# Mikubill/sketch2img

Hardware: AMD Instinct MI355X
Metric: sketch-guided images/sec whole-node, SD1.5 512px 50-step DDIM (higher is better)
Workload: dtype fp16

## Files before the change

include/skg.h:

```cpp
#ifndef SKG_H_
#define SKG_H_

#include <stddef.h>
#include <stdint.h>

#ifdef __cplusplus
extern "C" {
#endif

#define SKG_OK 0
#define SKG_E_BADARG (-1)
#define SKG_E_UNSUPPORTED (-2)
#define SKG_E_LAUNCH (-3)

#define SKG_ABI_VERSION 6
int skg_abi_version(void);
const char* skg_last_error(void);

#define SKG_EPI_RELU 1u
#define SKG_EPI_OUT_F32 2u
#define SKG_EPI_GEGLU 4u
#define SKG_EPI_BIAS_ROWS 8u

int skg_gemm_f16(const void* A, int lda, const void* B, int ldb, void* C, void* C_lo, int ldc, int M, int N, int K,
// ... 90 lines not shown
                  float alpha, float beta, void* stream);
int skg_batch_copy_f16(const void* In, int ldi, int in_batch_rows, void* Out, int ldo, int out_batch_rows,
                       int batches, int rows_per_batch, int C, void* stream);
int skg_silu_f16(const void* X, int ldx, void* Y, int ldy, int M, int C, void* stream);
int skg_quick_gelu_f16(const void* X, int ldx, void* Y, int ldy, int M, int C, void* stream);
int skg_quick_gelu_bwd_f16(const void* F, int ldf, const void* dY, int lddy, void* out, int ldo, int M, int C, void* stream);
int skg_gelu_f16(const void* X, int ldx, void* Y, int ldy, int M, int C, void* stream);
int skg_sumpool2x2_f16(const void* X, int ldx, void* Y, int ldy, int rows, int H, int W, int C,
                       void* stream);
int skg_nchw_f32_to_nhwc_f16(const float* X, void* Y, int rows, int C, int HW, int Cpad, void* stream);
int skg_nhwc_f16_to_nchw_f32(const void* X, int ldx, float* Y, int rows, int C, int HW, void* stream);

typedef struct {
  const float* P;
  int s;
  int pad_;
} SkgLgpTap;
int skg_lgp_layer0_gather(const SkgLgpTap* taps, int ntaps, const void* Wextra, int ldw,
                          const void* bias0, const float* noise, float sigma, int samples,
                          void* Z, int rows, int h, int w, int H0, void* stream);
int skg_lgp_layer0_scatter(const void* dZ, int lddz, void* dP, int rows, int h, int w, int s, int H0,
                           void* stream);
size_t skg_bn_scratch_floats(int samples, int C);
int skg_bn_stats(const void* X, int ldx, int samples, int segs, int seg_rows, int C, float eps,
                 float* stats, float* scratch, float* running_mean, float* running_var,
                 void* stream);
int skg_bn_stats_from_running(const float* running_mean, const float* running_var, int samples,
                              int C, float eps, float* stats, void* stream);
int skg_bn_apply(const void* X, int ldx, void* Y, int ldy, int samples, int segs, int seg_rows,
                 int C, const float* stats, const void* gamma, const void* beta, void* stream);
int skg_bn_relu_bwd(const void* X, int ldx, const void* dY, int lddy, void* dX, int lddx,
                    int samples, int segs, int seg_rows, int C, const float* stats,
                    const void* gamma, int train_mode, float* scratch, void* stream);
int skg_lgp_mse_seed(const void* out, int ldo, const float* target, void* dOut, int ldd,
                     float* loss, int samples, int h, int w, float loss_scale, void* stream);

size_t skg_colsum_scratch_floats(int C);
int skg_colsum_f16(const void* X, int ldx, int M, int C, float scale, float* out, float* scratch, void* stream);
int skg_bn_param_grads(const void* X, int ldx, const void* dY, int lddy, int rows, int C, const float* stats,
                       float scale, float* dgamma, float* dbeta, float* scratch, void* stream);
int skg_lgp_extra_features(const float* noise, float sigma, int samples, int rows, int h, int w, void* E, int ld,
                           void* stream);
int skg_lgp_mse_train(const void* out, int ldo, const float* target, void* dOut, int ldd, float* loss_parts,
                      int samples, int h, float loss_scale, void* stream);
int skg_adamw_step(float* param, const float* grad, float* exp_avg, float* exp_avg_sq, void* param_f16, size_t n,
                   float lr, float beta1, float beta2, float eps, float weight_decay, int step, float inv_grad_scale,
                   void* stream);
int skg_nonfinite_flag(const float* x, size_t n, float* flag, int reset, void* stream);
int skg_adamw_step_guarded(float* param, const float* grad, float* exp_avg, float* exp_avg_sq, void* param_f16, size_t n,
                           float lr, float beta1, float beta2, float eps, float weight_decay, int step,
                           float inv_grad_scale, const float* skip_flag, void* stream);

int skg_cfg_ddim_step(const void* eps_u, const void* eps_c, int ld, int lo_off, const float* x, float* x_prev,
                      float* eps_out, int samples, int HW, float g, float c0, float c1, float c2,
                      float c3, int vpred, void* stream);
int skg_cfg_ddim_eta_step(const void* eps_u, const void* eps_c, int ld, int lo_off, const float* x, const float* z,
                          float* x_prev, float* eps_out, int samples, int HW, float g, float c0, float c1,
                          float c2, float c_dir, float sigma, int vpred, void* stream);
int skg_softmax_rows_f16(const void* x, int ldx, void* y, int ldy, int M, int N, void* stream);
int skg_image_postprocess(const void* x, int ld, float* out, size_t pixels, int C, float scale, float shift,
                          void* stream);

int skg_image_to_u8(const void* x, int ld, void* out, size_t pixels, int C, float scale, float shift, void* stream);

int skg_gaussian_sample(const void* moments, int ld, const float* noise, float* out, int samples, int L, int HW,
                        float scale, void* stream);
// ... 32 lines not shown
```

sketch2img_amd/_lib.py:

```python
from __future__ import annotations

import ctypes
import os

import torch

_HERE = os.path.dirname(os.path.abspath(__file__))
LIB_PATH = os.environ.get("SKG_LIB") or os.path.join(_HERE, "libskg.so")

ABI_VERSION = 6

SIGNATURES = {
    "skg_abi_version": ("i", ""),
    "skg_last_error": ("s", ""),
    "skg_gemm_f16": ("i", "pipippiiiipppifupiip"),
    "skg_conv3x3_up2_f16": ("i", "pipppiiiiiiipp"),
    "skg_conv3x3_sc_f16": ("i", "pipiipppiiiiiipupip"),
    "skg_conv4x4s2_f16": ("i", "pippiiiiiipp"),
    "skg_conv3x3_wino_v_bytes": ("z", "iiii"),
    "skg_conv3x3_wino_f16": ("i", "pippppiiiiiipppiup"),
    "skg_groupnorm_wino_fwd": ("i", "pipiiiiifppipp"),
    "skg_gemm_f16_rows": ("i", "pipipiiiipiip"),
    "skg_gemm_gn_fused": ("i", "iiiiiii"),
    "skg_gemm_f16_geglu_keep": ("i", "pipipipiiiipp"),
# ... 30 lines not shown
    "skg_bn_scratch_floats": ("z", "ii"),
    "skg_bn_stats": ("i", "piiiiifppppp"),
    "skg_bn_stats_from_running": ("i", "ppiifpp"),
    "skg_bn_apply": ("i", "pipiiiiipppp"),
    "skg_bn_relu_bwd": ("i", "pipipiiiiippipp"),
    "skg_colsum_scratch_floats": ("z", "i"),
    "skg_colsum_f16": ("i", "piiifppp"),
    "skg_bn_param_grads": ("i", "pipiiipfpppp"),
    "skg_lgp_extra_features": ("i", "pfiiiipip"),
    "skg_lgp_mse_train": ("i", "pippipiifp"),
    "skg_adamw_step": ("i", "pppppzfffffifp"),
    "skg_lgp_mse_seed": ("i", "pippipiiifp"),
    "skg_cfg_ddim_step": ("i", "ppiipppiifffffip"),
    "skg_cfg_ddim_eta_step": ("i", "ppiippppiiffffffip"),
    "skg_softmax_rows_f16": ("i", "pipiiip"),
    "skg_image_postprocess": ("i", "pipziffp"),
    "skg_image_to_u8": ("i", "pipziffp"),
    "skg_gaussian_sample": ("i", "pippiiifp"),
    "skg_cfg_dpmpp2m_step": ("i", "ppiippppiiffffffip"),
    "skg_guidance_update": ("i", "pipppiifp"),
    "skg_box_probe_mfma": ("i", "pip"),
    "skg_instnorm_scratch_floats": ("z", "iii"),
    "skg_instnorm_act_f16": ("i", "piiiifipifpifpp"),
    "skg_convt4x4s2_f16": ("i", "pippiiiiiipip"),
    "skg_a2s_patch_f16": ("i", "ppiiiip"),
    "skg_a2s_tail": ("i", "pippiiip"),
    "skg_wgrad_scratch_floats": ("z", "iii"),
    "skg_wgrad_f16": ("i", "pipiiiifipppp"),
    "skg_layernorm_param_scratch_floats": ("z", "i"),
    "skg_layernorm_param_grads": ("i", "pipiiipfipppp"),
    "skg_quick_gelu_bwd_f16": ("i", "pipipiiip"),
    "skg_nonfinite_flag": ("i", "pzpip"),
    "skg_adamw_step_guarded": ("i", "pppppzfffffifpp"),
}

_CT = {"p": ctypes.c_void_p, "i": ctypes.c_int, "f": ctypes.c_float, "u": ctypes.c_uint,
       "z": ctypes.c_size_t, "s": ctypes.c_char_p}


class SkgTap(ctypes.Structure):
    _fields_ = [("P", ctypes.c_void_p), ("s", ctypes.c_int), ("pad_", ctypes.c_int)]


class SkgError(RuntimeError):
    rc = 0


def _load():
    if not os.path.exists(LIB_PATH):
        raise ImportError(
            f"{LIB_PATH} not found: build it with `python -c 'import __graft_entry__ as g; g.build()'` "
            "or `make -C sketch2img_amd/csrc`.  sketch2img_amd has no fallback compute path.")
    lib = ctypes.CDLL(LIB_PATH)
    for name, (ret, args) in SIGNATURES.items():
        try:
            fn = getattr(lib, name)
        except AttributeError as e:
            raise ImportError(f"libskg.so does not export {name}") from e
        fn.restype = _CT[ret]
        fn.argtypes = [_CT[a] for a in args]
    if lib.skg_abi_version() != ABI_VERSION:
        raise ImportError(f"{LIB_PATH}: ABI version {lib.skg_abi_version()}, this package binds version {ABI_VERSION} "
                          "(include/skg.h SKG_ABI_VERSION) - rebuild with `make -C sketch2img_amd/csrc`")
    return lib


# ... 13 lines not shown
```

sketch2img_amd/csrc/lgp.hip:

```cpp
#include "common.h"

namespace {

constexpr int BN_CHUNKS = 64;
constexpr int MAX_TAPS = 12;
constexpr int NEXTRA = 40;

struct TapArgs {
  const float* P[MAX_TAPS];
  int s[MAX_TAPS];
  int n;
};

__device__ __forceinline__ void bil_coord(int d, int s, int h, int& i0, int& i1, float& w1) {
  const float scale = (float)s / (float)h;
  float src = ((float)d + 0.5f) * scale - 0.5f;
  if (src < 0.f) src = 0.f;
  i0 = (int)src;
  if (i0 > s - 1) i0 = s - 1;
  i1 = i0 + (i0 < s - 1 ? 1 : 0);
  w1 = src - (float)i0;
}

__global__ __launch_bounds__(256) void lgp_gather_kernel(const TapArgs taps, const half_t* __restrict__ Wx, int ldw,
// ... 548 lines not shown
    v[i] = vi;
    float w = p[i] * (1.f - lr * wd);
    w -= lr * (mi / bc1) / (sqrtf(vi / bc2) + eps);
    p[i] = w;
    if (p16) p16[i] = (half_t)w;
  }
}

__device__ __forceinline__ unsigned nonfinite_bits(unsigned u) { return (u & 0x7f800000u) == 0x7f800000u; }
__device__ __forceinline__ unsigned nonfinite_bits(const uint4& u) {
  return nonfinite_bits(u.x) | nonfinite_bits(u.y) | nonfinite_bits(u.z) | nonfinite_bits(u.w);
}

__global__ __launch_bounds__(256) void nonfinite_flag_kernel(const unsigned* __restrict__ x, size_t n, size_t head,
                                                             size_t nvec, float* __restrict__ flag) {
  const uint4* __restrict__ xv = reinterpret_cast<const uint4*>(x + head);
  const size_t stride = (size_t)gridDim.x * 256;
  size_t i = (size_t)blockIdx.x * 256 + threadIdx.x;
  unsigned bad = 0;
  for (; i + 3 * stride < nvec; i += 4 * stride) {
    const uint4 a = xv[i], b = xv[i + stride], c = xv[i + 2 * stride], d = xv[i + 3 * stride];
    bad |= nonfinite_bits(a) | nonfinite_bits(b) | nonfinite_bits(c) | nonfinite_bits(d);
  }
  for (; i < nvec; i += stride) bad |= nonfinite_bits(xv[i]);
  if (blockIdx.x == 0) {
    const size_t body_end = head + 4 * nvec;
    if (threadIdx.x < head) bad |= nonfinite_bits(x[threadIdx.x]);
    if (threadIdx.x >= 64 && body_end + (threadIdx.x - 64) < n) bad |= nonfinite_bits(x[body_end + (threadIdx.x - 64)]);
  }
  const unsigned long long hits = __ballot(bad != 0);
  if (hits != 0 && (threadIdx.x & 63) == 0) *flag = 1.0f;
}

inline int ew_grid(size_t total_items) {
  size_t b = (total_items + 255) / 256;
  if (b > 4096) b = 4096;
  if (b < 1) b = 1;
  return (int)b;
}

}

static inline bool tap_fits(int s, int h, int w) {
  return s > 0 && h % s == 0 && ((long long)s * w) % h == 0 && w % (int)((long long)s * w / h) == 0;
}

static inline bool grid_ok(int h, int w) { return h == w || (h % GT == 0 && w % GT == 0); }

extern "C" int skg_lgp_layer0_gather(const SkgLgpTap* taps, int ntaps, const void* Wextra, int ldw, const void* bias0,
                                     const float* noise, float sigma, int samples, void* Z, int rows, int h, int w, int H0,
                                     void* stream) {
  SKG_REQUIRE(grid_ok(h, w));
  SKG_REQUIRE(taps && ntaps > 0 && ntaps <= MAX_TAPS && bias0 && noise && Z && rows > 0 && h > 0 && w > 0);
  SKG_REQUIRE(H0 % 4 == 0 && skg_aligned(Z, 8) && samples > 0 && rows % samples == 0);
  SKG_REQUIRE(Wextra ? (ldw % 8 == 0 && skg_aligned(Wextra, 16)) : (h % GT == 0 && w % GT == 0 && H0 % GC == 0));
  TapArgs a{};
  a.n = ntaps;
  for (int i = 0; i < ntaps; ++i) {
    SKG_REQUIRE(taps[i].P && tap_fits(taps[i].s, h, w) && skg_aligned(taps[i].P, 16));
    a.P[i] = taps[i].P;
    a.s[i] = taps[i].s;
  }
  if (h % GT == 0 && w % GT == 0 && H0 % GC == 0) {
    hipLaunchKernelGGL(lgp_gather_tiled_kernel, dim3((h / GT) * (w / GT), rows, H0 / GC), dim3(256), 0,
                       (hipStream_t)stream, a, (const half_t*)Wextra, ldw, (const half_t*)bias0, noise, sigma, samples,
                       (half_t*)Z, rows, h, w, H0);
// ... 73 lines not shown
extern "C" int skg_bn_apply(const void* X, int ldx, void* Y, int ldy, int samples, int segs, int seg_rows, int C,
                            const float* stats, const void* gamma, const void* beta, void* stream) {
  SKG_REQUIRE(X && Y && stats && gamma && beta && samples > 0 && C % 8 == 0 && ldx % 8 == 0 && ldy % 8 == 0);
  SKG_REQUIRE(skg_aligned(X, 16) && skg_aligned(Y, 16) && skg_aligned(gamma, 16) && skg_aligned(beta, 16));
  SKG_REQUIRE(segs > 0 && seg_rows > 0);
  hipLaunchKernelGGL((bn_apply_kernel<0>), dim3(bn_apply_chunks(segs * seg_rows, C), samples), dim3(256), 0, (hipStream_t)stream,
                     (const half_t*)X, ldx, (const half_t*)nullptr, 0, (half_t*)Y, ldy, samples, segs, seg_rows, C,
                     stats, (const float*)nullptr, (const half_t*)gamma, (const half_t*)beta, 1);
  SKG_CHECK_LAUNCH("skg_bn_apply");
  return SKG_OK;
}

extern "C" int skg_bn_relu_bwd(const void* X, int ldx, const void* dY, int lddy, void* dX, int lddx, int samples,
                               int segs, int seg_rows, int C, const float* stats, const void* gamma,
                               int train_mode, float* scratch, void* stream) {
  SKG_REQUIRE(X && dY && dX && stats && gamma && scratch && samples > 0 && C % 8 == 0);
  SKG_REQUIRE(ldx % 8 == 0 && lddy % 8 == 0 && lddx % 8 == 0 && skg_aligned(X, 16) && skg_aligned(dY, 16) &&
              skg_aligned(dX, 16) && skg_aligned(gamma, 16));
  hipStream_t st = (hipStream_t)stream;
  float* sums = scratch + (size_t)samples * BN_CHUNKS * C * 2;
  if (train_mode) {
    hipLaunchKernelGGL((bn_partial_kernel<1>), dim3(BN_CHUNKS, samples), dim3(256), 0, st, (const half_t*)X, ldx,
                       (const half_t*)dY, lddy, samples, segs, seg_rows, C, stats, scratch);
    hipLaunchKernelGGL((bn_finalize_kernel<1>), dim3(skg_cdiv(C, 128), samples), dim3(128), 0, st, scratch, samples, C,
                       segs * seg_rows, 0.f, sums, (float*)nullptr);
  }
  hipLaunchKernelGGL((bn_apply_kernel<1>), dim3(bn_apply_chunks(segs * seg_rows, C), samples), dim3(256), 0, st, (const half_t*)X, ldx,
                     (const half_t*)dY, lddy, (half_t*)dX, lddx, samples, segs, seg_rows, C, stats, sums,
                     (const half_t*)gamma, (const half_t*)nullptr, train_mode);
  SKG_CHECK_LAUNCH("skg_bn_relu_bwd");
  return SKG_OK;
}

extern "C" size_t skg_colsum_scratch_floats(int C) { return (size_t)CS_CHUNKS * C; }

extern "C" int skg_colsum_f16(const void* X, int ldx, int M, int C, float scale, float* out, float* scratch,
                              void* stream) {
  SKG_REQUIRE(X && out && scratch && M > 0 && C > 0 && C % 8 == 0 && ldx % 8 == 0 && ldx >= C && skg_aligned(X, 16));
  hipStream_t st = (hipStream_t)stream;
  hipLaunchKernelGGL(colsum_partial_kernel, dim3(C / 8, CS_CHUNKS), dim3(256), 0, st, (const half_t*)X, ldx, M, C,
                     scratch);
  hipLaunchKernelGGL(colsum_final_kernel, dim3(skg_cdiv(C, 128)), dim3(128), 0, st, scratch, C, scale, out);
  SKG_CHECK_LAUNCH("skg_colsum_f16");
  return SKG_OK;
}

extern "C" int skg_bn_param_grads(const void* X, int ldx, const void* dY, int lddy, int rows, int C,
                                  const float* stats, float scale, float* dgamma, float* dbeta, float* scratch,
                                  void* stream) {
  SKG_REQUIRE(X && dY && stats && dgamma && dbeta && scratch && rows > 0 && C % 8 == 0 && ldx % 8 == 0 && lddy % 8 == 0 &&
              skg_aligned(X, 16) && skg_aligned(dY, 16));
  hipStream_t st = (hipStream_t)stream;
  hipLaunchKernelGGL((bn_partial_kernel<1>), dim3(BN_CHUNKS, 1), dim3(256), 0, st, (const half_t*)X, ldx,
                     (const half_t*)dY, lddy, 1, 1, rows, C, stats, scratch);
  hipLaunchKernelGGL(bn_param_grads_kernel, dim3(skg_cdiv(C, 128)), dim3(128), 0, st, scratch, C, scale, dgamma, dbeta);
  SKG_CHECK_LAUNCH("skg_bn_param_grads");
  return SKG_OK;
}

extern "C" int skg_lgp_mse_train(const void* out, int ldo, const float* target, void* dOut, int ldd,
                                 float* loss_parts, int samples, int h, float loss_scale, void* stream) {
  SKG_REQUIRE(out && target && dOut && loss_parts && samples > 0 && h > 0 && ldo >= 4 && ldd >= 4 && ldo % 4 == 0 &&
              ldd % 4 == 0 && skg_aligned(out, 8) && skg_aligned(dOut, 8));
  if (hipMemsetAsync(dOut, 0, (size_t)samples * h * h * ldd * sizeof(half_t), (hipStream_t)stream) != hipSuccess)
    return SKG_E_LAUNCH;
  hipLaunchKernelGGL(mse_train_kernel, dim3(samples), dim3(256), 0, (hipStream_t)stream, (const half_t*)out, ldo,
// ... 41 lines not shown
```

sketch2img_amd/lgp.py:

```python
from __future__ import annotations

from typing import Dict, List, Optional, Sequence, Tuple

import torch

from . import ops

LIN = (0, 3, 6, 9, 12)
BNS = (2, 5, 8, 11)
OUT_PAD = 8
SEED_LD = 32
LOSS_SCALE = 4096.0


class HipLGP:
    def __init__(self, state_dict: Dict[str, torch.Tensor], tap_channels: Sequence[int], device="cuda",
                 training: bool = True):
        dev = self.dev = torch.device(device)
        self.training = training
        self.tap_channels = list(tap_channels)
        self.E = sum(tap_channels)
        h16 = lambda t: t.detach().to(dev, torch.float16).contiguous()
        f32 = lambda t: t.detach().to(dev, torch.float32).contiguous()
        w0 = state_dict["layers.0.weight"]
        assert w0.shape[1] == self.E + 40, "LGP input_dim must be sum(tap channels) + 4 + 36"
        self.H0 = w0.shape[0]
        self.W0 = h16(w0)
        self.W0T = h16(w0[:, : self.E].t())
        self.W0x = h16(torch.nn.functional.pad(w0[:, self.E:], (0, 64 - 40)))
        self.b = [h16(state_dict[f"layers.{i}.bias"]) for i in LIN]
        self.W = [self.W0] + [h16(state_dict[f"layers.{i}.weight"]) for i in LIN[1:]]
        self.WT = [None] + [h16(state_dict[f"layers.{i}.weight"].t()) for i in LIN[1:]]
        w4 = state_dict["layers.12.weight"]
        self.out_dim = w4.shape[0]
        assert self.out_dim <= OUT_PAD
        self.W[4] = h16(torch.nn.functional.pad(w4, (0, 0, 0, OUT_PAD - self.out_dim)))
        self.b[4] = h16(torch.nn.functional.pad(state_dict["layers.12.bias"], (0, OUT_PAD - self.out_dim)))
        self.WT[4] = h16(torch.nn.functional.pad(w4.t(), (0, SEED_LD - self.out_dim)))
        self.gamma = [h16(state_dict[f"layers.{i}.weight"]) for i in BNS]
        self.beta = [h16(state_dict[f"layers.{i}.bias"]) for i in BNS]
        self.running_mean = [f32(state_dict[f"layers.{i}.running_mean"]) for i in BNS]
        self.running_var = [f32(state_dict[f"layers.{i}.running_var"]) for i in BNS]
        self.num_batches_tracked = [int(state_dict[f"layers.{i}.num_batches_tracked"]) for i in BNS]

    def forward(self, taps: Sequence[Tuple[torch.Tensor, int]], noise: torch.Tensor, sigma: float, S: int,
                h: int, keep: Optional[dict] = None, w: Optional[int] = None) -> torch.Tensor:
        w = h if w is None else w
        wk = None if w == h else w
        hw = h * w
        P, sizes, off = [], [], 0
        for (F, s), C in zip(taps, self.tap_channels):
            s = s if isinstance(s, int) else s[0]
            assert F.shape == (2 * S * s * (s * w // h), C)
            P.append(ops.gemm(F, self.W0[:, off:off + C], out_f32=True))
            sizes.append(s)
            off += C
        if h % 8 == 0 and w % 8 == 0 and self.H0 % 128 == 0:
            Ex = ops.lgp_extra_features(noise, sigma, S, 2 * S, h, 64, w=wk)
            Z = ops.lgp_layer0_gather(P + [ops.gemm(Ex, self.W0x, out_f32=True)], sizes + [h], None, self.b[0], noise,
                                      sigma, S, h, self.H0, w=wk)
        else:
            Z = ops.lgp_layer0_gather(P, sizes, self.W0[:, self.E:], self.b[0], noise, sigma, S, h, self.H0, w=wk)
        zs, stats = [], []
        for l in range(4):
            if self.training:
                st = ops.bn_stats(Z, S, 2, hw, 1e-5, self.running_mean[l], self.running_var[l])
                self.num_batches_tracked[l] += S
            else:
                st = ops.bn_stats_from_running(self.running_mean[l], self.running_var[l], S)
            A = ops.bn_apply(Z, S, 2, hw, st, self.gamma[l], self.beta[l])
            zs.append(Z)
            stats.append(st)
            Z = ops.gemm(A, self.W[l + 1], bias=self.b[l + 1], relu=(l < 3))
        if keep is not None:
            keep.update(zs=zs, stats=stats, sizes=sizes, S=S, h=h, w=w)
        return Z

    def backward(self, out: torch.Tensor, target: torch.Tensor, keep: dict):
        S, h, zs, stats, sizes = keep["S"], keep["h"], keep["zs"], keep["stats"], keep["sizes"]
        w = keep.get("w", h)
        wk = None if w == h else w
        hw = h * w
        dOut, loss = ops.lgp_mse_seed(out, target, S, h, SEED_LD, LOSS_SCALE, w=wk)
        dA = ops.gemm(dOut, self.WT[4])
        dZ = None
        for l in (3, 2, 1, 0):
            dZ = ops.bn_relu_bwd(zs[l], dA, S, 2, hw, stats[l], self.gamma[l], self.training)
            if l > 0:
                dA = ops.gemm(dZ, self.WT[l])
        dZc = dZ[S * hw:]
        grads, off = [], 0
        for s, C in zip(sizes, self.tap_channels):
            dP = ops.lgp_layer0_scatter(dZc, S, h, s, self.H0, w=wk)
            grads.append(ops.gemm(dP, self.W0T[off:off + C]))
            off += C
        return grads, loss

    def state_dict(self) -> Dict[str, torch.Tensor]:
        sd = {}
        for l, i in enumerate(BNS):
            sd[f"layers.{i}.running_mean"] = self.running_mean[l].clone()
            sd[f"layers.{i}.running_var"] = self.running_var[l].clone()
            sd[f"layers.{i}.num_batches_tracked"] = torch.tensor(self.num_batches_tracked[l])
        return sd
```

sketch2img_amd/ops.py:

```python
from __future__ import annotations

import ctypes
import threading
from typing import List, Optional, Sequence, Tuple

import torch

from ._lib import SkgError, SkgTap, check, lib

EPI_RELU, EPI_OUT_F32, EPI_GEGLU, EPI_BIAS_ROWS = 1, 2, 4, 8
CONV_S1, CONV_S2, CONV_UP2, CONV_S2T, CONV_S2A = 0, 1, 2, 3, 4
ATTN_CAUSAL, ATTN_ROWV, ATTN_RESIDENT_KV = 1, 2, 4


_workspace = {}
_workspace_lock = threading.Lock()
WORKSPACE_BYTES = 128 << 20
_capture_owner = None


def _stream() -> int:
    st = torch.cuda.current_stream()
    key = (st.device.index, st.cuda_stream)
    if key not in _workspace:
# ... 695 lines not shown
          "skg_bn_stats")
    return stats


def bn_stats_from_running(running_mean, running_var, samples, eps=1e-5):
    C = running_mean.numel()
    stats = torch.empty(samples, C, 2, device=running_mean.device, dtype=torch.float32)
    check(lib.skg_bn_stats_from_running(_p(running_mean), _p(running_var), samples, C, eps, _p(stats), _stream()),
          "skg_bn_stats_from_running")
    return stats


def bn_apply(X, samples, segs, seg_rows, stats, gamma, beta, out=None):
    _f16(X, gamma, beta)
    C = X.shape[1]
    if out is None:
        out = torch.empty(X.shape[0], C, device=X.device, dtype=torch.float16)
    check(lib.skg_bn_apply(_p(X), _ld(X), _p(out), _ld(out), samples, segs, seg_rows, C, _p(stats), _p(gamma),
                           _p(beta), _stream()), "skg_bn_apply")
    return out


def bn_relu_bwd(X, dY, samples, segs, seg_rows, stats, gamma, train: bool, out=None):
    _f16(X, dY, gamma)
    C = X.shape[1]
    if out is None:
        out = torch.empty(X.shape[0], C, device=X.device, dtype=torch.float16)
    check(lib.skg_bn_relu_bwd(_p(X), _ld(X), _p(dY), _ld(dY), _p(out), _ld(out), samples, segs, seg_rows, C,
                              _p(stats), _p(gamma), int(train), _p(_bn_scratch(samples, C, X.device)), _stream()),
          "skg_bn_relu_bwd")
    return out


def lgp_mse_seed(out16, target, samples, h, ldd, loss_scale, w: Optional[int] = None):
    _f16(out16)
    wd = h if w is None else w
    dOut = torch.empty(2 * samples * h * wd, ldd, device=out16.device, dtype=torch.float16)
    loss = torch.empty(samples, device=out16.device, dtype=torch.float32)
    check(lib.skg_lgp_mse_seed(_p(out16), _ld(out16), _p(target), _p(dOut), ldd, _p(loss), samples, h, wd,
                               loss_scale, _stream()), "skg_lgp_mse_seed")
    return dOut, loss


def colsum(X, scale: float = 1.0):
    _f16(X)
    M, C = X.shape
    out = torch.empty(C, device=X.device, dtype=torch.float32)
    scr = _scratch_buf(("colsum", _skey(X.device), C), lib.skg_colsum_scratch_floats(C), X.device)
    check(lib.skg_colsum_f16(_p(X), _ld(X), M, C, scale, _p(out), _p(scr), _stream()), "skg_colsum_f16")
    return out


def bn_param_grads(X, dY, stats, scale: float = 1.0):
    _f16(X, dY)
    M, C = X.shape
    dg = torch.empty(C, device=X.device, dtype=torch.float32)
    db = torch.empty(C, device=X.device, dtype=torch.float32)
    check(lib.skg_bn_param_grads(_p(X), _ld(X), _p(dY), _ld(dY), M, C, _p(stats), scale, _p(dg), _p(db),
                                 _p(_bn_scratch(1, C, X.device)), _stream()), "skg_bn_param_grads")
    return dg, db


def lgp_extra_features(noise, sigma: float, samples: int, rows: int, h: int, ld: int = 64, w: Optional[int] = None):
    wd = h if w is None else w
    out = torch.empty(rows * h * wd, ld, device=noise.device, dtype=torch.float16)
    check(lib.skg_lgp_extra_features(_p(noise), sigma, samples, rows, h, wd, _p(out), ld, _stream()),
# ... 202 lines not shown
```

Baseline: 6.030.

## Fuse LGP batchnorm apply, linear GEMM, and BN stats into single kernels

Adds an MFMA linear kernel that applies the previous layer's batchnorm (or its ReLU backward) as a prologue while staging A tiles, and accumulates per-sample BN statistics or backward sums in the epilogue, followed by a small finalize kernel. The forward and backward passes of the latent guidance predictor MLP use it by default instead of separate bn_stats/bn_apply/gemm/bn_relu_bwd launches, removing intermediate activation round-trips and kernel launches. It also deduplicates layer0 scatter for repeated tap sizes. The added scratch buffers and shape restrictions fall back to the old path when they are not met.

```diff
diff --git a/include/skg.h b/include/skg.h
--- a/include/skg.h
+++ b/include/skg.h
@@ -146,6 +146,20 @@
 int skg_bn_relu_bwd(const void* X, int ldx, const void* dY, int lddy, void* dX, int lddx,
                     int samples, int segs, int seg_rows, int C, const float* stats,
                     const void* gamma, int train_mode, float* scratch, void* stream);
+int skg_bn_relu_bwd_from_sums(const void* X, int ldx, const void* dY, int lddy, void* dX, int lddx,
+                              int samples, int segs, int seg_rows, int C, const float* stats,
+                              const float* sums, const void* gamma, int train_mode, void* stream);
+
+size_t skg_lgp_linear_scratch_floats(int M, int N);
+int skg_lgp_linear_bn_f16(const void* X, int ldx, const void* W, int ldw, const void* bias, void* Y, int ldy,
+                          int M, int N, int K, int samples, int seg_rows, const float* stats,
+                          const void* gamma, const void* beta, int relu, float* partial, float* stats_out,
+                          float eps, float* running_mean, float* running_var, void* stream);
+int skg_lgp_linear_bn_bwd_f16(const void* dY, int lddy, const void* Zp, int ldzp, const float* stats_p,
+                              const float* sums_p, const void* gamma_p, const void* WT, int ldw, void* dA,
+                              int ldda, int M, int N, int K, int samples, int seg_rows, int train_mode,
+                              const void* Z, int ldz, const float* stats, float* partial, float* sums_out,
+                              void* stream);
 int skg_lgp_mse_seed(const void* out, int ldo, const float* target, void* dOut, int ldd,
                      float* loss, int samples, int h, int w, float loss_scale, void* stream);
 
diff --git a/sketch2img_amd/_lib.py b/sketch2img_amd/_lib.py
--- a/sketch2img_amd/_lib.py
+++ b/sketch2img_amd/_lib.py
@@ -86,6 +86,10 @@
     "skg_quick_gelu_bwd_f16": ("i", "pipipiiip"),
     "skg_nonfinite_flag": ("i", "pzpip"),
     "skg_adamw_step_guarded": ("i", "pppppzfffffifpp"),
+    "skg_bn_relu_bwd_from_sums": ("i", "pipipiiiiipppip"),
+    "skg_lgp_linear_scratch_floats": ("z", "ii"),
+    "skg_lgp_linear_bn_f16": ("i", "pipippiiiiiipppippfppp"),
+    "skg_lgp_linear_bn_bwd_f16": ("i", "pipippppipiiiiiiipipppp"),
 }
 
 _CT = {"p": ctypes.c_void_p, "i": ctypes.c_int, "f": ctypes.c_float, "u": ctypes.c_uint,
diff --git a/sketch2img_amd/csrc/lgp.hip b/sketch2img_amd/csrc/lgp.hip
--- a/sketch2img_amd/csrc/lgp.hip
+++ b/sketch2img_amd/csrc/lgp.hip
@@ -604,6 +604,290 @@
   if (hits != 0 && (threadIdx.x & 63) == 0) *flag = 1.0f;
 }
 
+constexpr int LB_M = 128, LB_K = 32, LB_PITCH = 40;
+constexpr int LB_CF = 2048;
+constexpr int LB_SMAX = 32;
+
+struct LinArgs {
+  const half_t* A; int lda;
+  const half_t* X; int ldx;
+  const half_t* W; int ldw;
+  const half_t* bias;
+  half_t* C; int ldc;
+  int M, N, K, S, seg_rows, relu, train, epi;
+  const float* pstats;
+  const float* psums;
+  const half_t* gamma;
+  const half_t* beta;
+  float* partial;
+  const half_t* EX; int ldex;
+  const float* estats;
+};
+
+template <int BN, int PRO>
+__global__ __launch_bounds__(256) void lgp_linear_kernel(const LinArgs p) {
+  constexpr int WN = BN / 2, NT = WN / 16, MT = 4, BPT = BN / 64;
+  __shared__ __attribute__((aligned(16))) half_t As[2][LB_M * LB_PITCH];
+  __shared__ __attribute__((aligned(16))) half_t Bs[2][BN * LB_PITCH];
+  __shared__ __attribute__((aligned(16))) float cf[PRO ? LB_CF : 4];
+  __shared__ float red[4][WN][2];
+
+  const int tid = threadIdx.x;
+  const int lane = tid & 63, wave = tid >> 6;
+  const int wm = wave >> 1, wn = wave & 1;
+  const int g = lane >> 4, l16 = lane & 15;
+  const int m0 = blockIdx.y * LB_M, n0 = blockIdx.x * BN;
+  const int K = p.K;
+
+  int smp[2];
+#pragma unroll
+  for (int q = 0; q < 2; ++q) smp[q] = (min(m0 + 64 * q, p.M - 1) / p.seg_rows) % p.S;
+
+  if (PRO) {
+    for (int idx = tid; idx < 2 * K; idx += 256) {
+      const int q = idx / K, k = idx - q * K;
+      const int gs = smp[q];
+      const float mean = p.pstats[((size_t)gs * K + k) * 2], rstd = p.pstats[((size_t)gs * K + k) * 2 + 1];
+      const float a = (float)p.gamma[k] * rstd;
+      cf[(0 * 2 + q) * K + k] = a;
+      if (PRO == 1) {
+        cf[(1 * 2 + q) * K + k] = (float)p.beta[k] - mean * a;
+      } else {
+        const float m1 = p.train ? p.psums[((size_t)gs * K + k) * 2] : 0.f;
+        const float m2 = p.train ? p.psums[((size_t)gs * K + k) * 2 + 1] : 0.f;
+        const float c = a * rstd * m2;
+        cf[(2 * 2 + q) * K + k] = c;
+        cf[(1 * 2 + q) * K + k] = a * m1 - c * mean;
+      }
+    }
+  }
+
+  const int lrow = tid >> 2;
+  const int lkc = (tid & 3) * 8;
+  bool a_ok[2];
+  size_t a_off[2], x_off[2];
+#pragma unroll
+  for (int q = 0; q < 2; ++q) {
+    const int m = m0 + lrow + 64 * q;
+    a_ok[q] = m < p.M;
+    a_off[q] = (size_t)(a_ok[q] ? m : 0) * p.lda + lkc;
+    x_off[q] = PRO == 2 ? (size_t)(a_ok[q] ? m : 0) * p.ldx + lkc : 0;
+  }
+  bool b_ok[BPT];
+  const half_t* b_base[BPT];
+#pragma unroll
+  for (int q = 0; q < BPT; ++q) {
+    const int n = n0 + lrow + 64 * q;
+    b_ok[q] = n < p.N;
+    b_base[q] = p.W + (size_t)(b_ok[q] ? n : 0) * p.ldw + lkc;
+  }
+
+  half8_t ra[2], rx[2], rb[BPT];
+  auto load_tiles = [&](int kt) {
+    const int k0 = kt * LB_K;
+#pragma unroll
+    for (int q = 0; q < 2; ++q) {
+      ra[q] = a_ok[q] ? ld_half8(p.A + a_off[q] + k0) : zero_half8();
+      if (PRO == 2) rx[q] = a_ok[q] ? ld_half8(p.X + x_off[q] + k0) : zero_half8();
+    }
+#pragma unroll
+    for (int q = 0; q < BPT; ++q) rb[q] = b_ok[q] ? ld_half8(b_base[q] + k0) : zero_half8();
+  };
+  auto store_tiles = [&](int buf, int kt) {
+    const int k = kt * LB_K + lkc;
+#pragma unroll
+    for (int q = 0; q < 2; ++q) {
+      half8_t o = ra[q];
+      if (PRO == 1) {
+        const float* ca = &cf[(0 * 2 + q) * K + k];
+        const float* cb = &cf[(1 * 2 + q) * K + k];
+#pragma unroll
+        for (int j = 0; j < 8; ++j) {
+          const float x = (float)ra[q][j];
+          o[j] = (half_t)(x * ca[j] + cb[j]);
+        }
+      } else if (PRO == 2) {
+        const float* ca = &cf[(0 * 2 + q) * K + k];
+        const float* cb = &cf[(1 * 2 + q) * K + k];
+        const float* cc = &cf[(2 * 2 + q) * K + k];
+#pragma unroll
+        for (int j = 0; j < 8; ++j) {
+          const float x = (float)rx[q][j];
+          o[j] = x > 0.f ? (half_t)((float)ra[q][j] * ca[j] - cb[j] - x * cc[j]) : (half_t)0.f;
+        }
+      }
+      st_half8(&As[buf][(lrow + 64 * q) * LB_PITCH + lkc], o);
+    }
+#pragma unroll
+    for (int q = 0; q < BPT; ++q) st_half8(&Bs[buf][(lrow + 64 * q) * LB_PITCH + lkc], rb[q]);
+  };
+
+  float4_t acc[MT][NT];
+#pragma unroll
+  for (int i = 0; i < MT; ++i)
+#pragma unroll
+    for (int j = 0; j < NT; ++j) acc[i][j] = float4_t{0.f, 0.f, 0.f, 0.f};
+
+  const int KT = K / LB_K;
+  load_tiles(0);
+  if (PRO) __syncthreads();
+  store_tiles(0, 0);
+  __syncthreads();
+  for (int kt = 0; kt < KT; ++kt) {
+    const int cur = kt & 1;
+    const bool more = kt + 1 < KT;
+    if (more) load_tiles(kt + 1);
+    half8_t xf[MT], wf[NT];
+#pragma unroll
+    for (int i = 0; i < MT; ++i) xf[i] = ld_half8(&As[cur][(wm * 64 + i * 16 + l16) * LB_PITCH + g * 8]);
+#pragma unroll
+    for (int j = 0; j < NT; ++j) wf[j] = ld_half8(&Bs[cur][(wn * WN + j * 16 + l16) * LB_PITCH + g * 8]);
+#pragma unroll
+    for (int i = 0; i < MT; ++i)
+#pragma unroll
+      for (int j = 0; j < NT; ++j)
+        acc[i][j] = __builtin_amdgcn_mfma_f32_16x16x32_f16(wf[j], xf[i], acc[i][j], 0, 0, 0);
+    if (more) store_tiles(cur ^ 1, kt + 1);
+    __syncthreads();
+  }
+
+  float s1[NT][4], s2[NT][4];
+#pragma unroll
+  for (int j = 0; j < NT; ++j)
+#pragma unroll
+    for (int e = 0; e < 4; ++e) { s1[j][e] = 0.f; s2[j][e] = 0.f; }
+  const int gs = smp[wm];
+#pragma unroll
+  for (int j = 0; j < NT; ++j) {
+    const int n = n0 + wn * WN + j * 16 + g * 4;
+    if (n >= p.N) continue;
+    float bz[4] = {0.f, 0.f, 0.f, 0.f}, mu[4] = {0.f, 0.f, 0.f, 0.f}, rs[4] = {0.f, 0.f, 0.f, 0.f};
+    if (p.bias) {
+      const half4_t b = ld_half4(p.bias + n);
+#pragma unroll
+      for (int e = 0; e < 4; ++e) bz[e] = (float)b[e];
+    }
+    if (p.epi == 2) {
+#pragma unroll
+      for (int e = 0; e < 4; ++e) {
+        mu[e] = p.estats[((size_t)gs * p.N + n + e) * 2];
+        rs[e] = p.estats[((size_t)gs * p.N + n + e) * 2 + 1];
+      }
+    }
+#pragma unroll
+    for (int i = 0; i < MT; ++i) {
+      const int m = m0 + wm * 64 + i * 16 + l16;
+      if (m >= p.M) continue;
+      float4_t v = acc[i][j];
+      v[0] += bz[0]; v[1] += bz[1]; v[2] += bz[2]; v[3] += bz[3];
+      if (p.relu) {
+        v[0] = fmaxf(v[0], 0.f); v[1] = fmaxf(v[1], 0.f); v[2] = fmaxf(v[2], 0.f); v[3] = fmaxf(v[3], 0.f);
+      }
+      const half4_t o = {(half_t)v[0], (half_t)v[1], (half_t)v[2], (half_t)v[3]};
+      st_half4(p.C + (size_t)m * p.ldc + n, o);
+      if (p.epi == 1) {
+#pragma unroll
+        for (int e = 0; e < 4; ++e) {
+          const float a = (float)o[e];
+          s1[j][e] += a; s2[j][e] += a * a;
+        }
+      } else if (p.epi == 2) {
+        const half4_t z = ld_half4(p.EX + (size_t)m * p.ldex + n);
+#pragma unroll
+        for (int e = 0; e < 4; ++e) {
+          const float d = (float)o[e];
+          s1[j][e] += d; s2[j][e] += d * ((float)z[e] - mu[e]) * rs[e];
+        }
+      }
+    }
+  }
+  if (!p.epi) return;
+#pragma unroll
+  for (int j = 0; j < NT; ++j)
+#pragma unroll
+    for (int e = 0; e < 4; ++e) {
+      float a = s1[j][e], b = s2[j][e];
+#pragma unroll
+      for (int o = 1; o < 16; o <<= 1) { a += __shfl_xor(a, o, 64); b += __shfl_xor(b, o, 64); }
+      if (l16 == 0) { red[wave][j * 16 + g * 4 + e][0] = a; red[wave][j * 16 + g * 4 + e][1] = b; }
+    }
+  __syncthreads();
+  if (tid < BN && n0 + tid < p.N) {
+    const int cw = tid / WN, cl = tid - cw * WN;
+    const bool one = m0 + 64 >= p.M || (m0 + 64) / p.seg_rows == m0 / p.seg_rows;
+    float* o = p.partial + (((size_t)blockIdx.y * 2) * p.N + n0 + tid) * 2;
+    const float a0 = red[cw][cl][0], a1 = red[cw][cl][1], b0 = red[2 + cw][cl][0], b1 = red[2 + cw][cl][1];
+    o[0] = one ? a0 + b0 : a0;
+    o[1] = one ? a1 + b1 : a1;
+    o[(size_t)p.N * 2] = one ? 0.f : b0;
+    o[(size_t)p.N * 2 + 1] = one ? 0.f : b1;
+  }
+}
+
+constexpr int LF_C = 16, LF_L = 16;
+template <int KIND>
+__global__ __launch_bounds__(LF_C * LF_L) void lgp_linear_finalize_kernel(const float* __restrict__ partial, int S, int segs,
+                                                                          int seg_rows, int C, float eps,
+                                                                          float* __restrict__ out,
+                                                                          float* __restrict__ running_mean,
+                                                                          float* __restrict__ running_var) {
+  __shared__ float ls[LB_SMAX][LF_L / 4][LF_C][2];
+  __shared__ float mv[LB_SMAX][LF_C][2];
+  const int cl = threadIdx.x % LF_C, ln = threadIdx.x / LF_C;
+  const int c = blockIdx.x * LF_C + cl;
+  const int n = segs * seg_rows;
+  const bool ok = c < C;
+  for (int gq = 0; gq < S; ++gq) {
+    float s1 = 0.f, s2 = 0.f;
+    for (int j = 0; ok && j < segs; ++j) {
+      const int seg = j * S + gq;
+      const int r0 = seg * seg_rows, r1 = r0 + seg_rows;
+      for (int t = r0 / LB_M + ln; t <= (r1 - 1) / LB_M; t += LF_L) {
+        const int slot = seg - (t * LB_M) / seg_rows;
+        const float2_t q = *reinterpret_cast<const float2_t*>(partial + (((size_t)t * 2 + slot) * C + c) * 2);
+        s1 += q[0]; s2 += q[1];
+      }
+    }
+    s1 += __shfl_xor(s1, 16, 64); s2 += __shfl_xor(s2, 16, 64);
+    s1 += __shfl_xor(s1, 32, 64); s2 += __shfl_xor(s2, 32, 64);
+    if ((ln & 3) == 0) { ls[gq][ln >> 2][cl][0] = s1; ls[gq][ln >> 2][cl][1] = s2; }
+  }
+  __syncthreads();
+  for (int gq = ln; ok && gq < S; gq += LF_L) {
+    float s1 = 0.f, s2 = 0.f;
+#pragma unroll
+    for (int l = 0; l < LF_L / 4; ++l) { s1 += ls[gq][l][cl][0]; s2 += ls[gq][l][cl][1]; }
+    if (KIND == 0) {
+      const float mean = s1 / n;
+      const float var = fmaxf(s2 / n - mean * mean, 0.f);
+      out[((size_t)gq * C + c) * 2] = mean;
+      out[((size_t)gq * C + c) * 2 + 1] = rsqrtf(var + eps);
+      mv[gq][cl][0] = mean; mv[gq][cl][1] = var;
+    } else {
+      out[((size_t)gq * C + c) * 2] = s1 / n;
+      out[((size_t)gq * C + c) * 2 + 1] = s2 / n;
+    }
+  }
+  if (KIND != 0 || running_mean == nullptr) return;
+  __syncthreads();
+  if (ok && ln == 0) {
+    float rm = running_mean[c], rv = running_var[c];
+    for (int gq = 0; gq < S; ++gq) {
+      rm = 0.9f * rm + 0.1f * mv[gq][cl][0];
+      rv = 0.9f * rv + 0.1f * mv[gq][cl][1] * ((float)n / (float)(n - 1));
+    }
+    running_mean[c] = rm;
+    running_var[c] = rv;
+  }
+}
+
+template <int PRO>
+inline void lgp_linear_launch(const LinArgs& a, hipStream_t st) {
+  const int tm = skg_cdiv(a.M, LB_M);
+  if (a.N % 128 == 0) hipLaunchKernelGGL((lgp_linear_kernel<128, PRO>), dim3(a.N / 128, tm), dim3(256), 0, st, a);
+  else hipLaunchKernelGGL((lgp_linear_kernel<64, PRO>), dim3(skg_cdiv(a.N, 64), tm), dim3(256), 0, st, a);
+}
+
 inline int ew_grid(size_t total_items) {
   size_t b = (total_items + 255) / 256;
   if (b > 4096) b = 4096;
@@ -743,6 +1027,88 @@
   return SKG_OK;
 }
 
+extern "C" int skg_bn_relu_bwd_from_sums(const void* X, int ldx, const void* dY, int lddy, void* dX, int lddx, int samples,
+                                         int segs, int seg_rows, int C, const float* stats, const float* sums,
+                                         const void* gamma, int train_mode, void* stream) {
+  SKG_REQUIRE(X && dY && dX && stats && gamma && (sums || !train_mode) && samples > 0 && segs > 0 && seg_rows > 0 && C > 0 &&
+              C % 8 == 0);
+  SKG_REQUIRE(ldx % 8 == 0 && lddy % 8 == 0 && lddx % 8 == 0 && skg_aligned(X, 16) && skg_aligned(dY, 16) &&
+              skg_aligned(dX, 16) && skg_aligned(gamma, 16));
+  hipLaunchKernelGGL((bn_apply_kernel<1>), dim3(bn_apply_chunks(segs * seg_rows, C), samples), dim3(256), 0,
+                     (hipStream_t)stream, (const half_t*)X, ldx, (const half_t*)dY, lddy, (half_t*)dX, lddx, samples, segs,
+                     seg_rows, C, stats, sums, (const half_t*)gamma, (const half_t*)nullptr, train_mode);
+  SKG_CHECK_LAUNCH("skg_bn_relu_bwd_from_sums");
+  return SKG_OK;
+}
+
+static inline int lgp_linear_shape(int M, int N, int K, int samples, int seg_rows, int kcap) {
+  SKG_REQUIRE(M > 0 && N > 0 && K > 0 && samples > 0 && seg_rows > 0 && K % 32 == 0 && N % 8 == 0);
+  SKG_REQUIRE(M % seg_rows == 0 && (M / seg_rows) % samples == 0);
+  if (seg_rows % 64 != 0 || K > kcap || samples > LB_SMAX) return SKG_E_UNSUPPORTED;
+  return SKG_OK;
+}
+
+extern "C" size_t skg_lgp_linear_scratch_floats(int M, int N) {
+  return M > 0 && N > 0 ? (size_t)skg_cdiv(M, LB_M) * 2 * N * 2 : 0;
+}
+
+extern "C" int skg_lgp_linear_bn_f16(const void* X, int ldx, const void* W, int ldw, const void* bias, void* Y, int ldy, int M,
+                                     int N, int K, int samples, int seg_rows, const float* stats, const void* gamma,
+                                     const void* beta, int relu, float* partial, float* stats_out, float eps,
+                                     float* running_mean, float* running_var, void* stream) {
+  SKG_REQUIRE(X && W && Y && (!stats || (gamma && beta)) && (!partial || stats_out));
+  SKG_REQUIRE((running_mean == nullptr) == (running_var == nullptr) && (partial || !running_mean));
+  if (const int rc = lgp_linear_shape(M, N, K, samples, seg_rows, LB_CF / 4)) return rc;
+  SKG_REQUIRE(ldx % 8 == 0 && ldw % 8 == 0 && ldy % 4 == 0 && ldx >= K && ldw >= K && ldy >= N && skg_aligned(X, 16) &&
+              skg_aligned(W, 16) && skg_aligned(Y, 8) && skg_aligned(bias, 8));
+  hipStream_t st = (hipStream_t)stream;
+  LinArgs a{};
+  a.A = (const half_t*)X; a.lda = ldx;
+  a.W = (const half_t*)W; a.ldw = ldw;
+  a.bias = (const half_t*)bias;
+  a.C = (half_t*)Y; a.ldc = ldy;
+  a.M = M; a.N = N; a.K = K; a.S = samples; a.seg_rows = seg_rows; a.relu = relu; a.train = 1; a.epi = partial ? 1 : 0;
+  a.pstats = stats; a.gamma = (const half_t*)gamma; a.beta = (const half_t*)beta;
+  a.partial = partial;
+  if (stats) lgp_linear_launch<1>(a, st);
+  else lgp_linear_launch<0>(a, st);
+  if (partial)
+    hipLaunchKernelGGL((lgp_linear_finalize_kernel<0>), dim3(skg_cdiv(N, LF_C)), dim3(LF_C * LF_L), 0, st, partial, samples,
+                       M / seg_rows / samples, seg_rows, N, eps, stats_out, running_mean, running_var);
+  SKG_CHECK_LAUNCH("skg_lgp_linear_bn_f16");
+  return SKG_OK;
+}
+
+extern "C" int skg_lgp_linear_bn_bwd_f16(const void* dY, int lddy, const void* Zp, int ldzp, const float* stats_p,
+                                         const float* sums_p, const void* gamma_p, const void* WT, int ldw, void* dA, int ldda,
+                                         int M, int N, int K, int samples, int seg_rows, int train_mode, const void* Z, int ldz,
+                                         const float* stats, float* partial, float* sums_out, void* stream) {
+  SKG_REQUIRE(dY && WT && dA && (!Zp || (stats_p && gamma_p && (sums_p || !train_mode))));
+  SKG_REQUIRE(!partial || (Z && stats && sums_out));
+  if (const int rc = lgp_linear_shape(M, N, K, samples, seg_rows, LB_CF / 8)) return rc;
+  SKG_REQUIRE(lddy % 8 == 0 && ldw % 8 == 0 && ldda % 4 == 0 && lddy >= K && ldw >= K && ldda >= N && skg_aligned(dY, 16) &&
+              skg_aligned(WT, 16) && skg_aligned(dA, 8));
+  SKG_REQUIRE(!Zp || (ldzp % 8 == 0 && ldzp >= K && skg_aligned(Zp, 16)));
+  SKG_REQUIRE(!partial || (ldz % 4 == 0 && ldz >= N && skg_aligned(Z, 8)));
+  hipStream_t st = (hipStream_t)stream;
+  LinArgs a{};
+  a.A = (const half_t*)dY; a.lda = lddy;
+  a.X = (const half_t*)Zp; a.ldx = ldzp;
+  a.W = (const half_t*)WT; a.ldw = ldw;
+  a.C = (half_t*)dA; a.ldc = ldda;
+  a.M = M; a.N = N; a.K = K; a.S = samples; a.seg_rows = seg_rows; a.train = train_mode; a.epi = partial ? 2 : 0;
+  a.pstats = stats_p; a.psums = sums_p; a.gamma = (const half_t*)gamma_p;
+  a.partial = partial;
+  a.EX = (const half_t*)Z; a.ldex = ldz; a.estats = stats;
+  if (Zp) lgp_linear_launch<2>(a, st);
+  else lgp_linear_launch<0>(a, st);
+  if (partial)
+    hipLaunchKernelGGL((lgp_linear_finalize_kernel<1>), dim3(skg_cdiv(N, LF_C)), dim3(LF_C * LF_L), 0, st, partial, samples,
+                       M / seg_rows / samples, seg_rows, N, 0.f, sums_out, (float*)nullptr, (float*)nullptr);
+  SKG_CHECK_LAUNCH("skg_lgp_linear_bn_bwd_f16");
+  return SKG_OK;
+}
+
 extern "C" size_t skg_colsum_scratch_floats(int C) { return (size_t)CS_CHUNKS * C; }
 
 extern "C" int skg_colsum_f16(const void* X, int ldx, int M, int C, float scale, float* out, float* scratch,
diff --git a/sketch2img_amd/lgp.py b/sketch2img_amd/lgp.py
--- a/sketch2img_amd/lgp.py
+++ b/sketch2img_amd/lgp.py
@@ -1,5 +1,6 @@
 from __future__ import annotations
 
+import os
 from typing import Dict, List, Optional, Sequence, Tuple
 
 import torch
@@ -18,6 +19,7 @@
                  training: bool = True):
         dev = self.dev = torch.device(device)
         self.training = training
+        self.fused = os.environ.get("SKG_LGP_FUSED", "1") != "0"
         self.tap_channels = list(tap_channels)
         self.E = sum(tap_channels)
         h16 = lambda t: t.detach().to(dev, torch.float16).contiguous()
@@ -37,6 +39,7 @@
         self.W[4] = h16(torch.nn.functional.pad(w4, (0, 0, 0, OUT_PAD - self.out_dim)))
         self.b[4] = h16(torch.nn.functional.pad(state_dict["layers.12.bias"], (0, OUT_PAD - self.out_dim)))
         self.WT[4] = h16(torch.nn.functional.pad(w4.t(), (0, SEED_LD - self.out_dim)))
+        self.widths = [self.H0] + [self.W[l].shape[0] for l in range(1, 5)]
         self.gamma = [h16(state_dict[f"layers.{i}.weight"]) for i in BNS]
         self.beta = [h16(state_dict[f"layers.{i}.bias"]) for i in BNS]
         self.running_mean = [f32(state_dict[f"layers.{i}.running_mean"]) for i in BNS]
@@ -62,16 +65,26 @@
         else:
             Z = ops.lgp_layer0_gather(P, sizes, self.W0[:, self.E:], self.b[0], noise, sigma, S, h, self.H0, w=wk)
         zs, stats = [], []
+        fused = self.fused and ops.lgp_fusable(S, hw, self.widths)
+        st = None
         for l in range(4):
+            if not self.training:
+                st = ops.bn_stats_from_running(self.running_mean[l], self.running_var[l], S)
+            elif l == 0 or not fused:
+                st = ops.bn_stats(Z, S, 2, hw, 1e-5, self.running_mean[l], self.running_var[l])
             if self.training:
-                st = ops.bn_stats(Z, S, 2, hw, 1e-5, self.running_mean[l], self.running_var[l])
                 self.num_batches_tracked[l] += S
-            else:
-                st = ops.bn_stats_from_running(self.running_mean[l], self.running_var[l], S)
-            A = ops.bn_apply(Z, S, 2, hw, st, self.gamma[l], self.beta[l])
             zs.append(Z)
             stats.append(st)
-            Z = ops.gemm(A, self.W[l + 1], bias=self.b[l + 1], relu=(l < 3))
+            if not fused:
+                A = ops.bn_apply(Z, S, 2, hw, st, self.gamma[l], self.beta[l])
+                Z = ops.gemm(A, self.W[l + 1], bias=self.b[l + 1], relu=(l < 3))
+            elif self.training and l < 3:
+                Z, st = ops.lgp_linear_bn(Z, self.W[l + 1], self.b[l + 1], S, hw, st, self.gamma[l], self.beta[l], True,
+                                          want_stats=True, running_mean=self.running_mean[l + 1],
+                                          running_var=self.running_var[l + 1])
+            else:
+                Z = ops.lgp_linear_bn(Z, self.W[l + 1], self.b[l + 1], S, hw, st, self.gamma[l], self.beta[l], l < 3)
         if keep is not None:
             keep.update(zs=zs, stats=stats, sizes=sizes, S=S, h=h, w=w)
         return Z
@@ -82,17 +95,28 @@
         wk = None if w == h else w
         hw = h * w
         dOut, loss = ops.lgp_mse_seed(out, target, S, h, SEED_LD, LOSS_SCALE, w=wk)
-        dA = ops.gemm(dOut, self.WT[4])
-        dZ = None
-        for l in (3, 2, 1, 0):
-            dZ = ops.bn_relu_bwd(zs[l], dA, S, 2, hw, stats[l], self.gamma[l], self.training)
-            if l > 0:
-                dA = ops.gemm(dZ, self.WT[l])
+        train = self.training
+        if self.fused and ops.lgp_fusable(S, hw, self.widths):
+            r = ops.lgp_linear_bn_bwd(dOut, self.WT[4], S, hw, train, Z=zs[3] if train else None, stats=stats[3])
+            dA, sums = r if train else (r, None)
+            for l in (3, 2, 1):
+                r = ops.lgp_linear_bn_bwd(dA, self.WT[l], S, hw, train, Zp=zs[l], stats_p=stats[l], sums_p=sums,
+                                          gamma_p=self.gamma[l], Z=zs[l - 1] if train else None, stats=stats[l - 1])
+                dA, sums = r if train else (r, None)
+            dZ = ops.bn_relu_bwd_from_sums(zs[0], dA, S, 2, hw, stats[0], sums, self.gamma[0], train)
+        else:
+            dA = ops.gemm(dOut, self.WT[4])
+            dZ = None
+            for l in (3, 2, 1, 0):
+                dZ = ops.bn_relu_bwd(zs[l], dA, S, 2, hw, stats[l], self.gamma[l], train)
+                if l > 0:
+                    dA = ops.gemm(dZ, self.WT[l])
         dZc = dZ[S * hw:]
-        grads, off = [], 0
+        grads, off, dPs = [], 0, {}
         for s, C in zip(sizes, self.tap_channels):
-            dP = ops.lgp_layer0_scatter(dZc, S, h, s, self.H0, w=wk)
-            grads.append(ops.gemm(dP, self.W0T[off:off + C]))
+            if s not in dPs:
+                dPs[s] = ops.lgp_layer0_scatter(dZc, S, h, s, self.H0, w=wk)
+            grads.append(ops.gemm(dPs[s], self.W0T[off:off + C]))
             off += C
         return grads, loss
 
diff --git a/sketch2img_amd/ops.py b/sketch2img_amd/ops.py
--- a/sketch2img_amd/ops.py
+++ b/sketch2img_amd/ops.py
@@ -751,6 +751,61 @@
     return out
 
 
+def bn_relu_bwd_from_sums(X, dY, samples, segs, seg_rows, stats, sums, gamma, train: bool, out=None):
+    _f16(X, dY, gamma)
+    C = X.shape[1]
+    if out is None:
+        out = torch.empty(X.shape[0], C, device=X.device, dtype=torch.float16)
+    check(lib.skg_bn_relu_bwd_from_sums(_p(X), _ld(X), _p(dY), _ld(dY), _p(out), _ld(out), samples, segs, seg_rows, C,
+                                        _p(stats), _p(sums), _p(gamma), int(train), _stream()), "skg_bn_relu_bwd_from_sums")
+    return out
+
+
+LGP_FUSED_MAX_K, LGP_FUSED_MAX_K_BWD, LGP_FUSED_MAX_SAMPLES = 512, 256, 32
+
+
+def lgp_fusable(samples: int, seg_rows: int, widths: Sequence[int]) -> bool:
+    return (seg_rows % 64 == 0 and 0 < samples <= LGP_FUSED_MAX_SAMPLES and all(k % 32 == 0 and k <= LGP_FUSED_MAX_K for k in widths[:-1])
+            and all(k <= LGP_FUSED_MAX_K_BWD for k in widths[1:]) and all(n % 8 == 0 for n in widths))
+
+
+def _lgp_linear_scratch(M, N, dev):
+    n = lib.skg_lgp_linear_scratch_floats(M, N)
+    return _scratch_buf(("lgplin", _skey(dev), n), n, dev)
+
+
+def lgp_linear_bn(X, W, bias, samples, seg_rows, stats, gamma, beta, relu: bool, want_stats: bool = False, eps=1e-5,
+                  running_mean=None, running_var=None, out=None):
+    _f16(X, W, bias, gamma, beta)
+    M, K = X.shape
+    N = W.shape[0]
+    if out is None:
+        out = torch.empty(M, N, device=X.device, dtype=torch.float16)
+    st_out = torch.empty(samples, N, 2, device=X.device, dtype=torch.float32) if want_stats else None
+    part = _lgp_linear_scratch(M, N, X.device) if want_stats else None
+    check(lib.skg_lgp_linear_bn_f16(_p(X), _ld(X), _p(W), _ld(W), _p(bias), _p(out), _ld(out), M, N, K, samples, seg_rows,
+                                    _p(stats), _p(gamma), _p(beta), int(relu), _p(part), _p(st_out), eps, _p(running_mean),
+                                    _p(running_var), _stream()), "skg_lgp_linear_bn_f16")
+    return (out, st_out) if want_stats else out
+
+
+def lgp_linear_bn_bwd(dY, WT, samples, seg_rows, train: bool, Zp=None, stats_p=None, sums_p=None, gamma_p=None, Z=None,
+                      stats=None, out=None):
+    _f16(dY, WT, Zp, gamma_p, Z)
+    M, K = dY.shape
+    N = WT.shape[0]
+    if out is None:
+        out = torch.empty(M, N, device=dY.device, dtype=torch.float16)
+    want = Z is not None
+    sums = torch.empty(samples, N, 2, device=dY.device, dtype=torch.float32) if want else None
+    part = _lgp_linear_scratch(M, N, dY.device) if want else None
+    check(lib.skg_lgp_linear_bn_bwd_f16(_p(dY), _ld(dY), _p(Zp), _ld(Zp) if Zp is not None else 0, _p(stats_p), _p(sums_p),
+                                        _p(gamma_p), _p(WT), _ld(WT), _p(out), _ld(out), M, N, K, samples, seg_rows,
+                                        int(train), _p(Z), _ld(Z) if want else 0, _p(stats), _p(part), _p(sums), _stream()),
+          "skg_lgp_linear_bn_bwd_f16")
+    return (out, sums) if want else out
+
+
 def lgp_mse_seed(out16, target, samples, h, ldd, loss_scale, w: Optional[int] = None):
     _f16(out16)
     wd = h if w is None else w
```

New measurement: 6.044, median of 6. About the same (+0.2%).
